# iden3/snarkjs

Measured on NVIDIA H100. Metric: groth16_proofs_per_sec, higher is better.
Workload: dtype u32x8 (256-bit modular integers, 32-bit limbs)

## Files before the change

snarkjs_b200/csrc/api.cu:

```cuda
#include <cstdio>
#include <cstdlib>
#include <cstring>
#include <string>
#include <vector>
#include <map>
#include <algorithm>
#include <mutex>
#include <future>
#include <thread>
#include <dlfcn.h>
#include <nccl.h>
#include <fcntl.h>
#include <unistd.h>
#include <sys/mman.h>
#include <sys/stat.h>
#include "../../include/snarkb200.h"
#include "ec.cuh"
#include "msm.cuh"
#include "msm_entry.h"
#include "fr_entry.h"

using namespace sb;
namespace sb { double calibrate(int what, cudaStream_t stream); extern int g_ntt_tile_log; }

// ... 272 lines not shown
        hex_to_mont<BnFq>("1", c->gen1.data()); hex_to_mont<BnFq>("2", c->gen1.data() + 32);
        hex_to_mont<BnFq>("1800deef121f1e76426a00665e5c4479674322d4f75edadd46debd5cd992f6ed", c->gen2.data());
        hex_to_mont<BnFq>("198e9393920d483a7260bfb731fb5d25f1aa493335a9e71297e485b7aef312c2", c->gen2.data() + 32);
        hex_to_mont<BnFq>("12c85ea5db8c6deb4aab71808dcb408fe3d1e7690c43d37b4ce6cc0166fa7daa", c->gen2.data() + 64);
        hex_to_mont<BnFq>("090689d0585ff075ec9e99ad690c3395bc4b313370b38ef355acdadcd122975b", c->gen2.data() + 96);
    } else {
        c->gen1.resize(96); c->gen2.resize(192);
        hex_to_mont<BlsFq>("17f1d3a73197d7942695638c4fa9ac0fc3688c4f9774b905a14e3a3f171bac586c55e83ff97a1aeffb3af00adb22c6bb", c->gen1.data());
        hex_to_mont<BlsFq>("08b3f481e3aaa0f1a09e30ed741d8ae4fcf5e095d5d00af600db18cb2c04b3edd03cc744a2888ae40caa232946c5e7e1", c->gen1.data() + 48);
        hex_to_mont<BlsFq>("024aa2b2f08f0a91260805272dc51051c6e47ad4fa403b02b4510b647ae3d1770bac0326a805bbefd48056c8c121bdb8", c->gen2.data());
        hex_to_mont<BlsFq>("13e02b6052719f607dacd3a088274f65596bd0d09920b61ab5da61bbdc7f5049334cf11213945d57e5ac7d055d042b7e", c->gen2.data() + 48);
        hex_to_mont<BlsFq>("0ce5d527727d6e118cc9cdc6da2e351aadfd9baa8cbdd3a76d429a695160d12c923ac9cc3baca289e193548608b82801", c->gen2.data() + 96);
        hex_to_mont<BlsFq>("0606c4a02ea734cc32acd2b02bc28b99cb3e287e85a763af267492ab572e99ab3f370d275cec1da1aaa9075ff05f79be", c->gen2.data() + 144);
    }
}

void prof_begin(sb_ctx* c) { c->stats.ev = c->prof_ev; c->stats.nev = 256; c->stats.used = 0; for (double& d : c->stat) d = 0; }
void prof_end(sb_ctx* c) {
    for (int i = 0; i + 1 < c->stats.used; i += 2) {
        float ms = 0; if (cudaEventElapsedTime(&ms, c->prof_ev[i], c->prof_ev[i + 1]) != cudaSuccess) { cudaGetLastError(); continue; }
        const int g = c->stats.tag[i / 2];
        if (g == PROF_ACC_G1) { c->stat[0] += ms; c->stat[2] += 1; c->stat[9] += ms; }
        else if (g == PROF_ACC_G2) { c->stat[1] += ms; c->stat[3] += 1; c->stat[10] += ms; }
        else if (g == PROF_SORT) c->stat[8] += ms;
        else if (g >= PROF_FOLD && g <= PROF_JOIN) c->stat[11 + (g - PROF_FOLD)] += ms;
    }
    c->stats.ev = nullptr; c->stats.used = 0;
}

int g_serial_prove = 0;
int g_no_tables = 0;
int g_msm_chunk_log = 0;

bool want_precomp(sb_ctx* c, uint64_t n) {
    if (g_no_tables || n < (1ull << 12)) return false;
    MsmGeom g = msm_geometry_precomp(n, 32, c->fr_bits);
    return (uint64_t)g.W * n < (1ull << 31);
}
int build_table(sb_ctx* c, const GroupOps& G, const void* d_bases, uint64_t n, void** table, MsmGeom* gp) {
    MsmGeom g = msm_geometry_precomp(n, 32, c->fr_bits);
    cudaError_t e = cudaMalloc(table, (size_t)g.W * n * G.aff_bytes);
    if (e != cudaSuccess) { *table = nullptr; return cuda_fail(c, e, "precompute table allocation"); }
    int rc = G.precompute(d_bases, n, g.c, g.W, *table, c->stream); c->launches++;
    if (rc) return cuda_fail(c, (cudaError_t)rc, "k_precompute");
    e = cudaStreamSynchronize(c->stream);
    if (e != cudaSuccess) return cuda_fail(c, e, "k_precompute");
    *gp = g;
    return 0;
}

void tick(sb_ctx* c, int i) { cudaEventRecord(c->ev[i], c->stream); }
float elapsed(sb_ctx* c, int a, int b) { float ms = 0; cudaEventElapsedTime(&ms, c->ev[a], c->ev[b]); return ms; }

int msm_dev_accumulate(sb_ctx* c, const GroupOps& G, const void* d_bases, const uint8_t* d_scalars, uint32_t sbytes, uint64_t n,
                       uint8_t* acc_xyzz, const MsmGeom* gp = nullptr, uint64_t first = 0) {
    const uint64_t MAXC = 1ull << (g_msm_chunk_log > 0 ? g_msm_chunk_log : 23);
    for (uint64_t off = 0; off < n; off += MAXC) {
        uint64_t cn = std::min(MAXC, n - off);
        MsmGeom g = msm_geometry(cn, sbytes, c->fr_bits);
        if (gp) {
            g = *gp; g.first = first + off; g.W = (int)((8 * sbytes + 1 + g.c - 1) / g.c);
        }
        MsmSorted s;
        int rc = msm_sort_entries(d_scalars + off * sbytes, sbytes, cn, g, c->sort_scratch, c->stream, &s, &c->stats);
        if (rc) return cuda_fail(c, (cudaError_t)rc, "msm_sort_entries");
        void* d_wsum = c->io[3].get((size_t)g.wsum_points() * G.xyzz_bytes);
// ... 75 lines not shown
    for (void* p : {k->tA, k->tB1, k->tB2, k->tC, k->tH, k->dA, k->dB1, k->dB2, k->dC, k->dH, (void*)k->d_rowptr, (void*)k->d_sig, k->d_coef, k->dW, k->dA_T, k->dB_T, k->dC_T, k->dTmp, k->dTmp2, k->dTmp3, k->dWsum})
        if (p) cudaFree(p);
    delete k;
}

template <class PR> static void fr_from_mont_bytes(const uint8_t* in, uint8_t* out) { Fp<PR> a; memcpy(&a, in, 32); a = Fp<PR>::from_mont(a); memcpy(out, &a, 32); }
template <class PR> static void fr_neg_mul_bytes(const uint8_t* r, const uint8_t* s, uint8_t* out) { Fp<PR> a, b; memcpy(&a, r, 32); memcpy(&b, s, 32); a = Fp<PR>::neg(Fp<PR>::mul(a, b)); memcpy(out, &a, 32); }

}

extern "C" {

const char* sb_version(void) { return "snarkb200 0.2 (sm_90a)"; }
int sb_comm_destroy(sb_ctx* c);

int sb_create(int curve, int device_id, sb_ctx** out) {
    if (!out || (curve != SB_BN254 && curve != SB_BLS12_381)) return SB_ERR_ARG;
    int ndev = 0;
    if (cudaGetDeviceCount(&ndev) != cudaSuccess || ndev == 0) return SB_ERR_NODEVICE;
    if (device_id < 0 || device_id >= ndev) return SB_ERR_ARG;
    if (cudaSetDevice(device_id) != cudaSuccess) return SB_ERR_CUDA;
    sb_ctx* c = new sb_ctx();
    c->curve = curve; c->device = device_id;
    c->n8q = curve == SB_BN254 ? 32 : 48;
    c->fr_bits = curve == SB_BN254 ? 254 : 255;
    if (curve == SB_BN254) { c->g1 = SB_GROUP_OPS(bn254_g1, 64); c->g2 = SB_GROUP_OPS(bn254_g2, 128); }
    else { c->g1 = SB_GROUP_OPS(bls12381_g1, 96); c->g2 = SB_GROUP_OPS(bls12381_g2, 192); }
    if (cudaStreamCreate(&c->stream) != cudaSuccess) { delete c; return SB_ERR_CUDA; }
    for (auto& e : c->ev) cudaEventCreate(&e);
    for (auto& e : c->prof_ev) cudaEventCreate(&e);
    for (auto& e : c->pev) cudaEventCreateWithFlags(&e, cudaEventDisableTiming);
    { int lo = 0, hi = 0; cudaDeviceGetStreamPriorityRange(&lo, &hi);
      for (auto& st : c->aux) cudaStreamCreateWithPriority(&st, cudaStreamDefault, hi); }
    if (cudaHostAlloc((void**)&c->pinned, 256 * 1024, cudaHostAllocDefault) != cudaSuccess) c->pinned = nullptr;
    for (int i = 0; i < 2; i++) { if (cudaHostAlloc((void**)&c->stage[i], STAGE_BYTES, cudaHostAllocDefault) != cudaSuccess) c->stage[i] = nullptr; cudaEventCreateWithFlags(&c->stage_ev[i], cudaEventDisableTiming); }
    init_generators(c);
    int rc = curve == SB_BN254 ? init_roots<BnFr>(c) : init_roots<BlsFr>(c);
    if (rc == 0 && fr_configure(curve) != 0) rc = SB_ERR_CUDA;
    if (rc) { sb_destroy(c); return rc; }
    *out = c;
    return SB_OK;
}

void sb_destroy(sb_ctx* c) {
    if (!c) return;
    sb_comm_destroy(c);
    cudaSetDevice(c->device);
    cudaStreamSynchronize(c->stream);
    for (auto* k : c->keys) if (k) free_key(k);
    for (auto* k : c->plonk_keys) if (k) plonk_free_key(k);
    for (auto* k : c->fflonk_keys) if (k) fflonk_free_key(k);
    for (auto& b : c->bases) { if (b.d) cudaFree(b.d); if (b.table) cudaFree(b.table); }
    for (auto* t : c->pre_cache) { t->lo.release(); t->hi.release(); delete t; }
    for (auto& kv : c->ntt_fwd) { kv.second.lo.release(); kv.second.hi.release(); }
    for (auto& kv : c->ntt_inv) { kv.second.lo.release(); kv.second.hi.release(); }
    for (auto& kv : c->ninv) kv.second.release();
    c->wr_fwd.release(); c->wr_inv.release();
    for (auto& b : c->io) b.release();
    c->sort_scratch.release(); c->bucket_scratch.release();
    for (auto& e : c->ev) cudaEventDestroy(e);
    for (auto& e : c->prof_ev) cudaEventDestroy(e);
    for (auto& e : c->pev) cudaEventDestroy(e);
    for (auto& st : c->aux) { if (st) { cudaStreamSynchronize(st); cudaStreamDestroy(st); } }
    if (c->pinned) cudaFreeHost(c->pinned);
    for (int i = 0; i < 2; i++) { if (c->stage[i]) cudaFreeHost(c->stage[i]); cudaEventDestroy(c->stage_ev[i]); }
    c->sort_scratch2.release(); for (auto& b : c->bscr) b.release();
    cudaStreamDestroy(c->stream);
// ... 320 lines not shown
    k->nCoef = ncoef;
    cudaError_t e = cudaSuccess;
    auto up = [&](void** d, const void* src, size_t bytes, size_t alloc) {
        if (e != cudaSuccess) return;
        e = cudaMalloc(d, alloc ? alloc : 16); if (e != cudaSuccess) return;
        if (bytes) e = cudaMemcpy(*d, src, bytes, cudaMemcpyHostToDevice);
    };
    k->shard = shard; k->n_shards = n_shards;
    sb_shard_range(nv, shard, n_shards, &k->wlo, &k->wcnt);
    sb_shard_range(n, shard, n_shards, &k->hlo, &k->hcnt);
    const uint64_t wlo = k->wlo, wcnt = k->wcnt, hlo = k->hlo, hcnt = k->hcnt;
    auto upsec = [&](void** d, uint32_t id, uint64_t off, uint64_t len) {
        if (e != cudaSuccess) return;
        e = cudaMalloc(d, len ? len : 16); if (e != cudaSuccess) return;
        e = zkey_to_device(c, src, secs, id, off, len, *d);
    };
    upsec(&k->dA, 5, wlo * sG1, wcnt * sG1);
    upsec(&k->dB1, 6, wlo * sG1, wcnt * sG1);
    upsec(&k->dB2, 7, wlo * sG2, wcnt * sG2);
    if (e == cudaSuccess) {
        const uint64_t np1 = (uint64_t)k->nPublic + 1;
        e = cudaMalloc(&k->dC, wcnt ? wcnt * sG1 : 16);
        if (e == cudaSuccess && wcnt) e = cudaMemset(k->dC, 0, wcnt * sG1);
        const uint64_t g0 = std::max(wlo, np1), g1 = wlo + wcnt;
        if (e == cudaSuccess && g1 > g0) e = zkey_to_device(c, src, secs, 8, (g0 - np1) * sG1, (g1 - g0) * sG1, (uint8_t*)k->dC + (g0 - wlo) * sG1);
    }
    upsec(&k->dH, 9, hlo * sG1, hcnt * sG1);
    up((void**)&k->d_rowptr, rowptr.data(), rowptr.size() * 8, rowptr.size() * 8);
    up((void**)&k->d_sig, sig.data(), (size_t)ncoef * 4, (size_t)ncoef * 4);
    up(&k->d_coef, coef.data(), (size_t)ncoef * 32, (size_t)ncoef * 32);
    up(&k->dW, nullptr, 0, (nv + 64) * 32);
    up(&k->dA_T, nullptr, 0, n * 32); up(&k->dB_T, nullptr, 0, n * 32); up(&k->dC_T, nullptr, 0, n * 32); up(&k->dTmp, nullptr, 0, n * 32);
    up(&k->dTmp2, nullptr, 0, n * 32); up(&k->dTmp3, nullptr, 0, n * 32);
    up(&k->dWsum, nullptr, 0, 8 * 80 * 4 * 96);
    if (e != cudaSuccess) { free_key(k); return cuda_fail(c, e, "sb_groth16_load upload"); }
    if (want_precomp(c, wcnt) && want_precomp(c, hcnt)) {
        int rc2 = build_table(c, c->g1, k->dA, wcnt, &k->tA, &k->gpW);
        if (!rc2) rc2 = build_table(c, c->g1, k->dB1, wcnt, &k->tB1, &k->gpW);
        if (!rc2) rc2 = build_table(c, c->g2, k->dB2, wcnt, &k->tB2, &k->gpW);
        if (!rc2) rc2 = build_table(c, c->g1, k->dC, wcnt, &k->tC, &k->gpW);
        if (!rc2) rc2 = build_table(c, c->g1, k->dH, hcnt, &k->tH, &k->gpH);
        if (rc2) { free_key(k); return rc2; }
    }
    c->keys.push_back(k);
    *handle = c->keys.size();
    return 0;
}

int sb_groth16_load(sb_ctx* c, const uint8_t* z, uint64_t zlen, uint64_t* handle) { SB_LOCK(c);
    if (!z) return SB_ERR_ARG;
    ZkeySource src; src.z = z; src.zlen = zlen; return groth16_load_impl(c, src, 0, 1, handle);
}
int sb_groth16_load_sharded(sb_ctx* c, const uint8_t* z, uint64_t zlen, int shard, int n_shards, uint64_t* handle) { SB_LOCK(c);
    if (!z) return SB_ERR_ARG;
    ZkeySource src; src.z = z; src.zlen = zlen; return groth16_load_impl(c, src, shard, n_shards, handle);
}

int sb_groth16_load_file(sb_ctx* c, const char* path, uint64_t* handle) { SB_LOCK(c);
    if (!c || !path) return SB_ERR_ARG;
    cudaSetDevice(c->device);
    FILE* f = fopen(path, "rb");
    if (!f) return fail(c, SB_ERR_FORMAT, std::string("cannot open ") + path);
    ZkeySource src; src.f = f;
    int rc = groth16_load_impl(c, src, 0, 1, handle);
    fclose(f);
    return rc;
}
// ... 172 lines not shown
                        if (qcnt) NC(c, nc, nc->Send((const uint8_t*)odd[j] + qlo * 32, qcnt * 32, ncclUint8, q, c->comm, c->stream));
                    }
                } else if (hcnt) NC(c, nc, nc->Recv((uint8_t*)odd[j] + hlo * 32, hcnt * 32, ncclUint8, o, c->comm, c->stream));
            }
            NC(c, nc, nc->GroupEnd());
        }
        if (hcnt) {
            ProfScope pj(&c->stats, PROF_JOIN, c->stream);
            rc = fr_join_abc(cv, (const uint8_t*)odd[0] + hlo * 32, (const uint8_t*)odd[1] + hlo * 32, (const uint8_t*)odd[2] + hlo * 32,
                             (uint8_t*)tmp + hlo * 32, hcnt, c->stream); c->launches++;
            pj.end();
            if (rc) return cuda_fail(c, (cudaError_t)rc, "fr_join_abc");
        }
        return 0;
    };
    const GroupOps& G1 = c->g1; const GroupOps& G2 = c->g2;
    uint8_t* pA = partials; uint8_t* pB1 = pA + G1.xyzz_bytes; uint8_t* pC = pB1 + G1.xyzz_bytes; uint8_t* pH = pC + G1.xyzz_bytes; uint8_t* pB2 = pH + G1.xyzz_bytes;
    memset(partials, 0, 4 * G1.xyzz_bytes + G2.xyzz_bytes);
    std::vector<uint8_t> sA(G1.xyzz_bytes, 0), rB1(G1.xyzz_bytes, 0);
    const uint64_t MAXC = 1ull << (g_msm_chunk_log > 0 ? g_msm_chunk_log : 23);
    const bool local = k->n_shards > 1;
    if (local && (shard != k->shard || n_shards != k->n_shards)) return fail(c, SB_ERR_ARG, "proving key was loaded for a different shard");
    const uint64_t wb = local ? 0 : wlo, hb = local ? 0 : hlo;
    const bool overlapped = wcnt <= MAXC && hcnt <= MAXC && wcnt > 0 && hcnt > 0 && c->pinned;
    if (dist && world > 1 && !overlapped) return fail(c, SB_ERR_ARG, "distributed proving needs at least one point per rank and shards of at most 2^23 points");
    if (overlapped) {
        const bool serial = g_serial_prove != 0;
        cudaStream_t s0 = c->stream;
        cudaStream_t sN = serial ? s0 : c->aux[5];
        MsmGeom gw = msm_geometry(wcnt, 32, c->fr_bits), gh = msm_geometry(hcnt, 32, c->fr_bits);
        const bool pre = k->tA != nullptr;
        if (pre) { gw = k->gpW; gw.first = wb; gh = k->gpH; gh.first = hb; }
        const size_t w1 = (size_t)gw.wsum_points() * G1.xyzz_bytes, w2 = (size_t)gw.wsum_points() * G2.xyzz_bytes, wh = (size_t)gh.wsum_points() * G1.xyzz_bytes;
        if (3 * w1 + w2 + wh + 64 > 256 * 1024 || 3 * w1 + w2 + wh > (size_t)8 * 80 * 4 * 96) return fail(c, SB_ERR_ARG, "window buffer too small");
        uint8_t* dws = (uint8_t*)k->dWsum; uint8_t* hws = c->pinned;
        uint64_t* hcounts = (uint64_t*)(c->pinned + 3 * w1 + w2 + wh);
        CU(c, cudaEventRecord(c->pev[0], s0));
        if (sN != s0) CU(c, cudaStreamWaitEvent(sN, c->pev[0], 0));
        cudaStream_t saved = c->stream; c->stream = sN;
        rc = run_qap_ntt();
        MsmSorted sh;
        if (!rc) { rc = msm_sort_entries((const uint8_t*)tmp + hlo * 32, 32, hcnt, gh, c->sort_scratch2, sN, &sh, &c->stats); if (rc) rc = cuda_fail(c, (cudaError_t)rc, "msm_sort_entries"); }
        c->stream = saved;
        if (rc) return rc;
        CU(c, cudaEventRecord(c->pev[1], sN));
        MsmSorted sw;
        rc = msm_sort_entries((const uint8_t*)k->dW + wlo * 32, 32, wcnt, gw, c->sort_scratch, s0, &sw, &c->stats);
        if (rc) return cuda_fail(c, (cudaError_t)rc, "msm_sort_entries");
        tick(c, 2);
        struct Job { const GroupOps* G; const void* bases; size_t off; size_t len; uint8_t* dst; int tag; const MsmSorted* srt; const MsmGeom* g; };
        Job jobs[5] = {{&G1, pre ? k->tA : (const void*)((const uint8_t*)k->dA + wb * G1.aff_bytes), 0, w1, pA, SB_G1, &sw, &gw},
                       {&G1, pre ? k->tB1 : (const void*)((const uint8_t*)k->dB1 + wb * G1.aff_bytes), w1, w1, pB1, SB_G1, &sw, &gw},
                       {&G2, pre ? k->tB2 : (const void*)((const uint8_t*)k->dB2 + wb * G2.aff_bytes), 3 * w1, w2, pB2, SB_G2, &sw, &gw},
                       {&G1, pre ? k->tC : (const void*)((const uint8_t*)k->dC + wb * G1.aff_bytes), 2 * w1, w1, pC, SB_G1, &sw, &gw},
                       {&G1, pre ? k->tH : (const void*)((const uint8_t*)k->dH + hb * G1.aff_bytes), 3 * w1 + w2, wh, pH, SB_G1, &sh, &gh}};
        for (int i = 0; i < 5; i++) {
            cudaStream_t st = serial ? s0 : c->aux[i];
            if (i == 4 && sN != s0) CU(c, cudaStreamWaitEvent(s0, c->pev[1], 0));
            c->stats.cur_tag = jobs[i].tag;
            rc = jobs[i].G->buckets(jobs[i].bases, *jobs[i].srt, c->bscr[i], s0, dws + jobs[i].off, &c->stats, st, c->pev[8 + i]);
            if (rc) return cuda_fail(c, (cudaError_t)rc, "msm_buckets");
            CU(c, cudaMemcpyAsync(hws + jobs[i].off, dws + jobs[i].off, jobs[i].len, cudaMemcpyDeviceToHost, st));
            if (i == 0) CU(c, cudaMemcpyAsync(&hcounts[0], sw.counts, 8, cudaMemcpyDeviceToHost, st));
            if (i == 4) CU(c, cudaMemcpyAsync(&hcounts[1], sh.counts, 8, cudaMemcpyDeviceToHost, st));
            CU(c, cudaEventRecord(c->pev[2 + i], st));
        }
        tick(c, 3);
        for (int i = 0; i < 5; i++) {
            CU(c, cudaEventSynchronize(c->pev[2 + i]));
            jobs[i].G->combine(hws + jobs[i].off, *jobs[i].g, jobs[i].dst);
            if (ps && i == 0) G1.times(pA, ps->sp, 32, sA.data());
            if (ps && i == 1) G1.times(pB1, ps->rp, 32, rB1.data());
        }
        if (!serial) { for (int i = 0; i < 5; i++) CU(c, cudaStreamWaitEvent(s0, c->pev[2 + i], 0)); CU(c, cudaStreamWaitEvent(s0, c->pev[1], 0)); }
        c->stat[4] += 3.0 * (double)hcounts[0] + (double)hcounts[1]; c->stat[5] += (double)hcounts[0];
    } else {
    rc = run_qap_ntt(); if (rc) return rc;
    tick(c, 2);
    for (uint64_t off = 0; off < wcnt; off += MAXC) {
        uint64_t cn = std::min(MAXC, wcnt - off), base = wb + off;
        MsmGeom g = msm_geometry(cn, 32, c->fr_bits);
        MsmSorted s;
        rc = msm_sort_entries((const uint8_t*)k->dW + (wlo + off) * 32, 32, cn, g, c->sort_scratch, c->stream, &s, &c->stats);
        if (rc) return cuda_fail(c, (cudaError_t)rc, "msm_sort_entries");
        uint8_t* ws = (uint8_t*)k->dWsum;
        size_t w1 = (size_t)g.wsum_points() * G1.xyzz_bytes, w2 = (size_t)g.wsum_points() * G2.xyzz_bytes;
        if (3 * w1 + w2 > (size_t)8 * 80 * 4 * 96) return fail(c, SB_ERR_ARG, "window buffer too small");
        c->stats.cur_tag = SB_G1;
        rc = G1.buckets((const uint8_t*)k->dA + base * G1.aff_bytes, s, c->bucket_scratch, c->stream, ws, &c->stats, nullptr, nullptr); if (rc) return cuda_fail(c, (cudaError_t)rc, "msm A");
        rc = G1.buckets((const uint8_t*)k->dB1 + base * G1.aff_bytes, s, c->bucket_scratch, c->stream, ws + w1, &c->stats, nullptr, nullptr); if (rc) return cuda_fail(c, (cudaError_t)rc, "msm B1");
        rc = G1.buckets((const uint8_t*)k->dC + base * G1.aff_bytes, s, c->bucket_scratch, c->stream, ws + 2 * w1, &c->stats, nullptr, nullptr); if (rc) return cuda_fail(c, (cudaError_t)rc, "msm C");
        c->stats.cur_tag = SB_G2;
        rc = G2.buckets((const uint8_t*)k->dB2 + base * G2.aff_bytes, s, c->bucket_scratch, c->stream, ws + 3 * w1, &c->stats, nullptr, nullptr); if (rc) return cuda_fail(c, (cudaError_t)rc, "msm B2");
        std::vector<uint8_t> hw(3 * w1 + w2);
        uint64_t entries = 0;
        CU(c, cudaMemcpyAsync(hw.data(), ws, hw.size(), cudaMemcpyDeviceToHost, c->stream));
        CU(c, cudaMemcpyAsync(&entries, s.counts, 8, cudaMemcpyDeviceToHost, c->stream));
        CU(c, cudaStreamSynchronize(c->stream));
        c->stat[4] += 3.0 * (double)entries; c->stat[5] += (double)entries;
        G1.combine(hw.data(), g, pA); G1.combine(hw.data() + w1, g, pB1); G1.combine(hw.data() + 2 * w1, g, pC); G2.combine(hw.data() + 3 * w1, g, pB2);
    }
    tick(c, 3);
    if (hcnt) {
        rc = msm_dev_accumulate(c, G1, (const uint8_t*)k->dH + hb * G1.aff_bytes, (const uint8_t*)tmp + hlo * 32, 32, hcnt, pH);
        if (rc) return rc;
    }
    if (ps) { G1.times(pA, ps->sp, 32, sA.data()); G1.times(pB1, ps->rp, 32, rB1.data()); }
    }
    if (ps) {
        G1.add(pC, pH); G1.add(pC, sA.data()); G1.add(pC, rB1.data());
        memset(pB1, 0, G1.xyzz_bytes); memset(pH, 0, G1.xyzz_bytes);
    }
    tick(c, 4);
    cudaEventSynchronize(c->ev[4]);
    prof_end(c);
    c->last_ms[0] = elapsed(c, 0, 4); c->last_ms[1] = elapsed(c, 0, 1); c->last_ms[2] = elapsed(c, 1, 2); c->last_ms[3] = elapsed(c, 2, 3); c->last_ms[4] = elapsed(c, 3, 4);
    return 0;
}


// ... 332 lines not shown
```

snarkjs_b200/csrc/msm.cuh:

```cuda
#pragma once
#include <cuda_runtime.h>
#include "ec.cuh"
#include "msm_geom.h"

namespace sb {

static constexpr int MSM_SEG = 32;
static constexpr int MSM_ACC_THREADS = 128;
static constexpr int MSM_RED_CHUNK = 16;
static constexpr uint32_t MSM_INVALID_KEY = 0xffffffffu;
static constexpr int MSM_COUNTS_SEG = 8;

extern int g_msm_force_c;

__host__ inline MsmGeom msm_choose(uint64_t n, uint32_t scalar_bytes, int fr_bits, bool precomp) {
    int eff = (int)(8 * scalar_bytes) < fr_bits ? (int)(8 * scalar_bytes) : fr_bits;
    int best_c = 3; double best = 1e300;
    for (int c = 3; c <= 22; c++) {
        int weff = (eff + 1 + c - 1) / c, top = eff + 1 - (weff - 1) * c;
        if (weff > 1 && top < c - 5) continue;
        double buckets = (precomp ? 1.0 : (double)weff) * (double)(1u << (c - 1));
        double cost = (double)weff * (double)n * 10.0 + buckets * 60.0;
        if (cost < best) { best = cost; best_c = c; }
    }
// ... 185 lines not shown
    for (uint32_t s = 16; s > 0; s >>= 1) {
        if (threadIdx.x < s) { XYZZ<F> a = load_vec(sm + threadIdx.x), b = load_vec(sm + threadIdx.x + s); a.add(b); store_vec(sm + threadIdx.x, a); }
        __syncwarp();
    }
    if (threadIdx.x == 0) store_vec(out + blockIdx.x, load_vec(sm));
}

template <class F> __device__ __noinline__ void padd(XYZZ<F>& a, const XYZZ<F>& b) { a.add(b); }

struct AxisJob { const void* in; void* out; uint64_t total; uint32_t S; uint32_t log_inner; };

template <class F>
__global__ void __launch_bounds__(128)
k_axis_sum(AxisJob j0, AxisJob j1) {
    const AxisJob j = blockIdx.y ? j1 : j0;
    const uint64_t gid = blockIdx.x * (uint64_t)blockDim.x + threadIdx.x;
    if (gid >= j.total) return;
    const uint64_t o = gid >> j.log_inner, i = gid & ((1ull << j.log_inner) - 1);
    const XYZZ<F>* p = (const XYZZ<F>*)j.in + ((o * j.S) << j.log_inner) + i;
    XYZZ<F> acc = load_vec(p);
#pragma unroll 1
    for (uint32_t s = 1; s < j.S; s++) { XYZZ<F> v = load_vec(p + ((uint64_t)s << j.log_inner)); acc.add(v); }
    store_vec((XYZZ<F>*)j.out + gid, acc);
}

template <class F> __device__ __forceinline__ XYZZ<F> shfl_down_pt(const XYZZ<F>& v, int d) {
    constexpr int NW32 = sizeof(XYZZ<F>) / 4;
    union U { XYZZ<F> p; uint32_t w[NW32]; __device__ U() {} };
    U a, r; a.p = v;
#pragma unroll
    for (int k = 0; k < NW32; k++) r.w[k] = __shfl_down_sync(0xffffffffu, a.w[k], d);
    return r.p;
}
template <class F> __device__ __forceinline__ void warp_weighted_sum(XYZZ<F> v, XYZZ<F>& T, XYZZ<F>& W) {
    const int lane = threadIdx.x & 31;
#pragma unroll 1
    for (int d = 1; d < 32; d <<= 1) { XYZZ<F> o = shfl_down_pt<F>(v, d); if (lane + d < 32) v.add(o); }
    T = v;
    XYZZ<F> x = lane ? v : XYZZ<F>::inf();
#pragma unroll 1
    for (int d = 16; d >= 1; d >>= 1) { XYZZ<F> o = shfl_down_pt<F>(x, d); if (lane < d) x.add(o); }
    W = x;
}
template <class F> __device__ __forceinline__ XYZZ<F> warp_sum(XYZZ<F> x) {
    const int lane = threadIdx.x & 31;
#pragma unroll 1
    for (int d = 16; d >= 1; d >>= 1) { XYZZ<F> o = shfl_down_pt<F>(x, d); if (lane < d) x.add(o); }
    return x;
}

template <class F>
__global__ void __launch_bounds__(128)
k_ws_chunks(const XYZZ<F>* __restrict__ vecR, uint32_t lenR, const XYZZ<F>* __restrict__ vecC, uint32_t lenC, uint32_t NW, XYZZ<F>* __restrict__ tw) {
    const uint32_t nR = (lenR + 31) / 32, nC = (lenC + 31) / 32, per = nR + nC;
    const uint32_t wid = blockIdx.x * (blockDim.x >> 5) + (threadIdx.x >> 5), lane = threadIdx.x & 31;
    if (wid >= NW * per) return;
    const uint32_t w = wid / per, jj = wid % per;
    const bool isR = jj < nR;
    const uint32_t j = isR ? jj : jj - nR, len = isR ? lenR : lenC, idx = j * 32 + lane;
    const XYZZ<F>* vec = (isR ? vecR : vecC) + (uint64_t)w * len;
    XYZZ<F> v = XYZZ<F>::inf();
    if (idx < len) v = load_vec(vec + idx);
    XYZZ<F> T, W;
    warp_weighted_sum<F>(v, T, W);
    if (lane == 0) { store_vec(tw + 2 * (uint64_t)wid, T); store_vec(tw + 2 * (uint64_t)wid + 1, W); }
}

template <class F>
__global__ void __launch_bounds__(128)
k_ws_final(const XYZZ<F>* __restrict__ tw, uint32_t nR, uint32_t nC, XYZZ<F>* __restrict__ out) {
    const uint32_t warp = threadIdx.x >> 5, lane = threadIdx.x & 31, per = nR + nC;
    const XYZZ<F>* base = tw + 2 * (uint64_t)blockIdx.x * per;
    const bool r_side = warp < 2;
    const uint32_t cnt = r_side ? nR : nC, off = r_side ? 0 : nR;
    XYZZ<F> v = XYZZ<F>::inf();
    if (lane < cnt) v = load_vec(base + 2 * (uint64_t)(off + lane) + (warp & 1));
    XYZZ<F>* o = out + 5 * (uint64_t)blockIdx.x;
    if ((warp & 1) == 0) {
        XYZZ<F> tot, res;
        warp_weighted_sum<F>(v, tot, res);
        if (lane == 0) { store_vec(o + (r_side ? 0 : 2), res); if (!r_side) store_vec(o + 4, tot); }
    } else {
        XYZZ<F> res = warp_sum<F>(v);
        if (lane == 0) store_vec(o + (r_side ? 1 : 3), res);
    }
}

template <class F>
__global__ void __launch_bounds__(128)
k_axis_tree(AxisJob j0, AxisJob j1) {
    const AxisJob j = blockIdx.y ? j1 : j0;
    const uint64_t wid = blockIdx.x * (uint64_t)(blockDim.x >> 5) + (threadIdx.x >> 5);
    const uint32_t lane = threadIdx.x & 31;
    if (wid >= j.total) return;
    const uint64_t o = wid >> j.log_inner, i = wid & ((1ull << j.log_inner) - 1);
    const XYZZ<F>* p = (const XYZZ<F>*)j.in + ((o * j.S) << j.log_inner) + i;
    XYZZ<F> acc = XYZZ<F>::inf();
#pragma unroll 1
    for (uint32_t s = lane; s < j.S; s += 32) { XYZZ<F> v = load_vec(p + ((uint64_t)s << j.log_inner)); acc.add(v); }
    acc = warp_sum<F>(acc);
    if (lane == 0) store_vec((XYZZ<F>*)j.out + wid, acc);
}

static constexpr int WS_COL_BITS = 10;
struct WsPlan {
    bool ok = false;
    int m = 0, er = 0, ec = 0;
    int levels = 0; int br[8] = {0}, bc[8] = {0};
    uint32_t lenR = 0, lenC = 0, nR = 0, nC = 0;
    size_t rowA = 0, rowB = 0, colA = 0, colB = 0, tw = 0;
    size_t elems() const { return rowA + rowB + colA + colB + tw + 8; }
};
__host__ inline WsPlan ws_plan(const MsmGeom& g) {
    WsPlan p; const int cbits = g.c - 1; const size_t NW = g.windows();
    if (cbits > 2 * WS_COL_BITS || cbits < 0) return p;
    p.ok = true;
    if (cbits > WS_COL_BITS) { p.m = WS_COL_BITS; p.er = p.m; p.ec = cbits - p.m; p.lenR = 1u << p.ec; p.lenC = 1u << p.m; }
    else { p.lenR = 0; p.lenC = g.B; }
    int rr = p.er, rc = p.ec;
    for (int l = 0; l < 2 && (rr > 0 || rc > 0); l++) {
        p.levels++;
        p.br[l] = l == 0 ? (rr < 3 ? rr : 3) : rr; p.bc[l] = l == 0 ? (rc < 3 ? rc : 3) : rc; rr -= p.br[l]; rc -= p.bc[l];
        const size_t orow = p.br[l] ? (NW * g.B) >> (p.er - rr) : 0, ocol = p.bc[l] ? (NW * g.B) >> (p.ec - rc) : 0;
        if (l & 1) { p.rowB = orow; p.colB = ocol; } else { p.rowA = orow; p.colA = ocol; }
    }
    p.nR = (p.lenR + 31) / 32; p.nC = (p.lenC + 31) / 32;
    p.tw = 2 * NW * (p.nR + p.nC);
    return p;
}
__host__ inline size_t msm_reduce_scratch_elems(const MsmGeom& g) {
    const uint32_t NW = g.windows();
    const uint32_t L = g.B < (uint32_t)MSM_RED_CHUNK ? g.B : MSM_RED_CHUNK;
    const uint32_t ctas_per_window = (g.B / L + 127) / 128;
    const size_t legacy = (size_t)2 * NW * ctas_per_window;
    const WsPlan p = ws_plan(g);
    return (p.ok && p.elems() > legacy) ? p.elems() : legacy;
}

template <class F>
__global__ void __launch_bounds__(128) k_precompute(const Affine<F>* __restrict__ bases, uint64_t n, int c, int W, Affine<F>* __restrict__ table) {
    uint64_t i = blockIdx.x * (uint64_t)blockDim.x + threadIdx.x;
    if (i >= n) return;
    Affine<F> a = load_vec(bases + i);
    store_vec(table + i, a);
    if (a.is_inf()) {
        for (int w = 1; w < W; w++) store_vec(table + (uint64_t)w * n + i, a);
        return;
    }
    XYZZ<F> p; p.x = a.x; p.y = a.y; p.zz = F::one(); p.zzz = F::one();
    for (int w = 1; w < W; w++) {
        for (int j = 0; j < c; j++) p = XYZZ<F>::dbl(p);
        Affine<F> o;
        if (p.is_inf()) { o.x = F::zero(); o.y = F::zero(); }
        else { F t = PairInvF(F::mul(p.zz, p.zzz)); o.x = F::mul(p.x, F::mul(t, p.zzz)); o.y = F::mul(p.y, F::mul(t, p.zz)); p.x = o.x; p.y = o.y; p.zz = F::one(); p.zzz = F::one(); }
        store_vec(table + (uint64_t)w * n + i, o);
    }
}

__host__ __device__ inline uint64_t splitmix64(uint64_t x) {
    x += 0x9E3779B97F4A7C15ull; x = (x ^ (x >> 30)) * 0xBF58476D1CE4E5B9ull; x = (x ^ (x >> 27)) * 0x94D049BB133111EBull; return x ^ (x >> 31);
// ... 86 lines not shown
        ProfScope prof(stats, stats ? stats->cur_tag : 0, stream);
        {
            const unsigned grid = (unsigned)((heads0 + MSM_ACC_THREADS - 1) / MSM_ACC_THREADS);
            constexpr int MINB = sizeof(F) > 32 ? 2 : 4;
            k_accumulate<F, MINB><<<grid, MSM_ACC_THREADS, 0, stream>>>(d_bases, s.keys, s.vals, s.counts, buckets, headsA, hkA);
            launches++;
        }
        prof.end();
        if (tail_stream && tail_stream != stream && ev_acc) {
            cudaEventRecord(ev_acc, stream); cudaStreamWaitEvent(tail_stream, ev_acc, 0); stream = tail_stream;
        }
        ProfScope pfold(stats, PROF_FOLD, stream);
        k_fold_short<F><<<(unsigned)((heads0 + MSM_ACC_THREADS - 1) / MSM_ACC_THREADS), MSM_ACC_THREADS, 0, stream>>>(
            headsA, hkA, hkM, s.counts, buckets); launches++;
        uint64_t m = heads0; int level = 1;
        XYZZ<F>* hin = headsA; uint32_t* kin = hkM; XYZZ<F>* hout = headsB; uint32_t* kout = hkB;
        while (true) {
            uint64_t threads = (m + MSM_SEG - 1) / MSM_SEG;
            k_fold<F><<<(unsigned)((threads + MSM_ACC_THREADS - 1) / MSM_ACC_THREADS), MSM_ACC_THREADS, 0, stream>>>(
                hin, kin, s.counts, level, buckets, hout, kout); launches++;
            if (m <= (uint64_t)MSM_SEG) break;
            m = threads; level++;
            XYZZ<F>* th = hin; hin = hout; hout = th; uint32_t* tk = kin; kin = kout; kout = tk;
            if (level >= 8) return (int)cudaErrorUnknown;
        }
        pfold.end();
    }
    if (!heads0 && tail_stream && tail_stream != stream && ev_acc) { cudaEventRecord(ev_acc, stream); cudaStreamWaitEvent(tail_stream, ev_acc, 0); stream = tail_stream; }
    ProfScope pred(stats, PROF_REDUCE, stream);
    const WsPlan wp = ws_plan(g);
    if (wp.ok && !g_msm_force_reduce) {
        XYZZ<F>* rowb[2] = {partials, partials + wp.rowA};
        XYZZ<F>* colb[2] = {partials + wp.rowA + wp.rowB, partials + wp.rowA + wp.rowB + wp.colA};
        XYZZ<F>* tw = partials + wp.rowA + wp.rowB + wp.colA + wp.colB;
        const XYZZ<F>* rin = buckets; const XYZZ<F>* cin = buckets;
        int rr = wp.er, rc = wp.ec;
        for (int l = 0; l < wp.levels; l++) {
            AxisJob jr{nullptr, nullptr, 0, 1, 0}, jc{nullptr, nullptr, 0, 1, 0};
            if (wp.br[l]) { rr -= wp.br[l]; jr = AxisJob{rin, rowb[l & 1], (uint64_t)nbuckets >> (wp.er - rr), 1u << wp.br[l], (uint32_t)rr}; rin = rowb[l & 1]; }
            if (wp.bc[l]) { rc -= wp.bc[l]; jc = AxisJob{cin, colb[l & 1], (uint64_t)nbuckets >> (wp.ec - rc), 1u << wp.bc[l], (uint32_t)wp.m}; cin = colb[l & 1]; }
            const uint64_t mx = jr.total > jc.total ? jr.total : jc.total;
            if (l == 0) k_axis_sum<F><<<dim3((unsigned)((mx + 127) / 128), 2), 128, 0, stream>>>(jr, jc);
            else k_axis_tree<F><<<dim3((unsigned)((mx + 3) / 4), 2), 128, 0, stream>>>(jr, jc);
            launches++;
        }
        const uint32_t per = wp.nR + wp.nC;
        k_ws_chunks<F><<<(NW * per + 3) / 4, 128, 0, stream>>>(wp.lenR ? rin : nullptr, wp.lenR, cin, wp.lenC, NW, tw); launches++;
        k_ws_final<F><<<NW, 128, 0, stream>>>(tw, wp.nR, wp.nC, d_wsum); launches++;
    } else {
        k_reduce<F><<<NW * ctas_per_window, red_threads, red_threads * sizeof(XYZZ<F>), stream>>>(buckets, g, partials, ctas_per_window); launches++;
        k_window_sum<F><<<NW, 32, 32 * sizeof(XYZZ<F>), stream>>>(partials, ctas_per_window, d_wsum); launches++;
    }
    pred.end();
    if (stats) stats->launches += launches;
    return (int)cudaGetLastError();
}

}
```

snarkjs_b200/csrc/msm_geom.h:

```cpp
#pragma once
#include <cstdint>
namespace sb {
struct MsmGeom {
    int c;
    int W;
    uint32_t B;
    int precomp = 0;
    uint64_t stride = 0, first = 0;
    uint32_t windows() const { return precomp ? 1u : (uint32_t)W; }
    uint32_t wsum_points() const { return 5u * windows(); }
};
}
```

snarkjs_b200/csrc/msm_sort.cu:

```cuda
#include <cub/device/device_radix_sort.cuh>
#include "msm.cuh"

namespace sb {

int g_msm_force_reduce = 0;
int g_msm_force_c = 0;

__global__ void k_digits(const uint8_t* __restrict__ scalars, uint32_t sbytes, uint64_t n, MsmGeom g,
                         uint32_t* __restrict__ keys, uint32_t* __restrict__ vals) {
    uint64_t i = blockIdx.x * (uint64_t)blockDim.x + threadIdx.x;
    if (i >= n) return;
    uint32_t w32[17];
    const uint8_t* s = scalars + i * sbytes;
    if (sbytes == 32 && ((uintptr_t)scalars & 15) == 0) {
        const uint4* p = reinterpret_cast<const uint4*>(s);
        uint4 a = __ldg(p), b = __ldg(p + 1);
        w32[0] = a.x; w32[1] = a.y; w32[2] = a.z; w32[3] = a.w; w32[4] = b.x; w32[5] = b.y; w32[6] = b.z; w32[7] = b.w;
#pragma unroll
        for (int k = 8; k < 17; k++) w32[k] = 0;
    } else {
#pragma unroll
        for (int k = 0; k < 17; k++) w32[k] = 0;
        for (uint32_t k = 0; k < sbytes; k++) w32[k >> 2] |= (uint32_t)s[k] << (8 * (k & 3));
    }
    const uint32_t cmask = (1u << g.c) - 1, half = 1u << (g.c - 1);
    uint32_t carry = 0;
    for (int w = 0; w < g.W; w++) {
        uint32_t bit = (uint32_t)w * g.c, wi = bit >> 5, sh = bit & 31;
        uint64_t two = (uint64_t)w32[wi] | ((uint64_t)(wi + 1 < 17 ? w32[wi + 1] : 0) << 32);
        uint32_t raw = ((uint32_t)(two >> sh) & cmask) + carry;
        uint32_t key, val = (uint32_t)i;
        if (raw > half) { raw = (1u << g.c) - raw; carry = 1; val |= 0x80000000u; } else carry = 0;
        if (g.precomp) { key = raw ? raw - 1 : MSM_INVALID_KEY; val = (uint32_t)((uint64_t)w * g.stride + g.first + i) | (val & 0x80000000u); }
        else key = raw ? (uint32_t)w * g.B + raw - 1 : MSM_INVALID_KEY;
        keys[(uint64_t)w * n + i] = key;
        vals[(uint64_t)w * n + i] = val;
    }
}

__global__ void k_count_valid(const uint32_t* __restrict__ keys, uint64_t total, uint64_t* __restrict__ out, uint32_t T, uint32_t seg_lo, uint64_t wave) {
    if (blockIdx.x | threadIdx.x) return;
    uint64_t lo = 0, hi = total;
    while (lo < hi) { uint64_t mid = (lo + hi) >> 1; if (keys[mid] == MSM_INVALID_KEY) hi = mid; else lo = mid + 1; }
    out[0] = lo;
    uint64_t seg = T;
    if (wave) {
        const uint64_t k = (lo + wave * T - 1) / (wave * T);
        if (k && k <= 3) seg = (lo + k * wave - 1) / (k * wave);
        if (seg < seg_lo) seg = seg_lo;
        if (seg > T) seg = T;
    }
    out[MSM_COUNTS_SEG] = seg;
    uint64_t m = (lo + seg - 1) / seg;
    out[1] = m;
    for (int l = 2; l < 8; l++) { m = (m <= MSM_SEG) ? 0 : (m + MSM_SEG - 1) / MSM_SEG; out[l] = m; }
}

int msm_sort_entries(const uint8_t* d_scalars, uint32_t sbytes, uint64_t n, MsmGeom g, MsmScratch& scratch,
                     cudaStream_t stream, MsmSorted* out, MsmLaunchStats* stats) {
    const uint64_t total = n * (uint64_t)g.W;
    const uint64_t nbuckets = (uint64_t)g.windows() * g.B;
    if (sbytes == 0 || sbytes > 64) return (int)cudaErrorInvalidValue;
    int key_bits = 1; while ((1ull << key_bits) < nbuckets) key_bits++;
    int end_bit = key_bits + 1 > 32 ? 32 : key_bits + 1;
    size_t sort_tmp = 0;
    cub::DoubleBuffer<uint32_t> kb(nullptr, nullptr), vb(nullptr, nullptr);
    cub::DeviceRadixSort::SortPairs(nullptr, sort_tmp, kb, vb, (uint64_t)total, 0, end_bit, stream);
    auto al = [](size_t x) { return (x + 255) & ~(size_t)255; };
    size_t o_keys0 = 0, o_keys1 = o_keys0 + al(total * 4), o_vals0 = o_keys1 + al(total * 4), o_vals1 = o_vals0 + al(total * 4);
    size_t o_tmp = o_vals1 + al(total * 4), o_counts = o_tmp + al(sort_tmp);
    uint8_t* base = (uint8_t*)scratch.get(o_counts + 256);
    if (!base) return (int)cudaErrorMemoryAllocation;
    uint32_t* keys0 = (uint32_t*)(base + o_keys0); uint32_t* keys1 = (uint32_t*)(base + o_keys1);
    uint32_t* vals0 = (uint32_t*)(base + o_vals0); uint32_t* vals1 = (uint32_t*)(base + o_vals1);
    uint64_t* counts = (uint64_t*)(base + o_counts);
    int launches = 0;
    ProfScope prof(stats, PROF_SORT, stream);
    k_digits<<<(unsigned)((n + 255) / 256), 256, 0, stream>>>(d_scalars, sbytes, n, g, keys0, vals0); launches++;
    kb = cub::DoubleBuffer<uint32_t>(keys0, keys1); vb = cub::DoubleBuffer<uint32_t>(vals0, vals1);
    cudaError_t e = cub::DeviceRadixSort::SortPairs(base + o_tmp, sort_tmp, kb, vb, (uint64_t)total, 0, end_bit, stream);
    if (e != cudaSuccess) return (int)e;
    launches += 2 + (end_bit + 7) / 8;
    uint32_t T = MSM_SEG;
// ... 16 lines not shown
```

Measured before the change: 34.09.

## Replace weighted window sum with per-bit bucket sums and cap segment waves

Replaces the two-kernel weighted running-sum bucket reduction (k_ws_chunks + k_ws_final) with a single k_bit_sums kernel. For each window it computes the total plus one partial sum per bucket-index bit, giving c points per window instead of 5. The host-side window-sum buffers grow to 512 KiB to hold the larger output, so the host must combine more points. Separately, when the sorted entry count exceeds three waves, the segment length is now sized to fill exactly three waves instead of staying at T, which changes accumulation load balance. A profiling script is also added.

```diff
diff --git a/profiles/prof_tail.py b/profiles/prof_tail.py
--- /dev/null
+++ b/profiles/prof_tail.py
@@ -0,0 +1,68 @@
+import collections
+import os
+import re
+import sys
+
+sys.path.insert(0, os.path.dirname(os.path.dirname(os.path.abspath(__file__))))
+import numpy as np
+import torch
+from torch.profiler import ProfilerActivity, profile
+
+import snarkjs_b200
+from snarkjs_b200 import groth16, synth
+from snarkjs_b200.curve import _ptr
+
+FOLD = ("k_fold_short", "k_fold")
+REDUCE = ("k_axis_sum", "k_axis_tree", "k_bit_sums", "k_ws_chunks", "k_ws_final", "k_reduce", "k_window_sum")
+
+
+def short_name(name: str) -> str:
+    m = re.search(r"(\w+)\s*(<|\()", re.sub(r"^void\s+", "", name))
+    base = m.group(1) if m else name[:60]
+    return base + (" [G2]" if "Fp2" in name else "")
+
+
+def main():
+    L = int(os.environ.get("LOGN", "20"))
+    c = snarkjs_b200.getCurveFromName("bn128")
+    c.lib.sb_set_tuning(2, 1)
+    pk = groth16.ProvingKey(synth.synth_groth16_zkey(c, L, seed=1), curve=c)
+    w = synth.chain_witness(c.r, L)
+    r = (5 * (1 << 256) % c.r).to_bytes(32, "little")
+    s = (7 * (1 << 256) % c.r).to_bytes(32, "little")
+    proof = np.empty(8 * c.n8q, np.uint8)
+
+    def prove():
+        c.check(c.lib.sb_groth16_prove(c.handle, pk.handle, _ptr(w), w.size // 32, r, s, _ptr(proof)))
+
+    for _ in range(3):
+        prove()
+    torch.cuda.synchronize()
+    with profile(activities=[ProfilerActivity.CUDA]) as prof:
+        prove()
+        torch.cuda.synchronize()
+    tot = collections.defaultdict(float)
+    cnt = collections.defaultdict(int)
+    for e in prof.events():
+        if e.device_type != torch.autograd.DeviceType.CUDA:
+            continue
+        k = short_name(e.name)
+        tot[k] += e.time_range.elapsed_us() / 1e3
+        cnt[k] += 1
+    if not tot:
+        raise SystemExit("torch.profiler recorded no CUDA kernels")
+    gpu = torch.cuda.get_device_name(0)
+    print(f"# {gpu}, Groth16 2^{L}, serialised, prove call {c.last_ms(0):.2f} ms (library events)")
+    print(f"{'kernel':<44}{'ms':>9}{'launches':>10}")
+    for k in sorted(tot, key=tot.get, reverse=True):
+        print(f"{k:<44}{tot[k]:9.3f}{cnt[k]:10d}")
+    print(f"{'total kernel time':<44}{sum(tot.values()):9.3f}{sum(cnt.values()):10d}")
+    for label, names in (("fold", FOLD), ("bucket_reduce", REDUCE)):
+        ms = sum(v for k, v in tot.items() if k.split(" ")[0] in names)
+        n = sum(v for k, v in cnt.items() if k.split(" ")[0] in names)
+        print(f"class {label:<38}{ms:9.3f}{n:10d}")
+    pk.release()
+
+
+if __name__ == "__main__":
+    main()
diff --git a/snarkjs_b200/csrc/api.cu b/snarkjs_b200/csrc/api.cu
--- a/snarkjs_b200/csrc/api.cu
+++ b/snarkjs_b200/csrc/api.cu
@@ -328,6 +328,8 @@
 int g_no_tables = 0;
 int g_msm_chunk_log = 0;
 
+static constexpr size_t WSUM_BYTES = 512 * 1024;
+
 bool want_precomp(sb_ctx* c, uint64_t n) {
     if (g_no_tables || n < (1ull << 12)) return false;
     MsmGeom g = msm_geometry_precomp(n, 32, c->fr_bits);
@@ -469,7 +471,7 @@
     for (auto& e : c->pev) cudaEventCreateWithFlags(&e, cudaEventDisableTiming);
     { int lo = 0, hi = 0; cudaDeviceGetStreamPriorityRange(&lo, &hi);
       for (auto& st : c->aux) cudaStreamCreateWithPriority(&st, cudaStreamDefault, hi); }
-    if (cudaHostAlloc((void**)&c->pinned, 256 * 1024, cudaHostAllocDefault) != cudaSuccess) c->pinned = nullptr;
+    if (cudaHostAlloc((void**)&c->pinned, WSUM_BYTES, cudaHostAllocDefault) != cudaSuccess) c->pinned = nullptr;
     for (int i = 0; i < 2; i++) { if (cudaHostAlloc((void**)&c->stage[i], STAGE_BYTES, cudaHostAllocDefault) != cudaSuccess) c->stage[i] = nullptr; cudaEventCreateWithFlags(&c->stage_ev[i], cudaEventDisableTiming); }
     init_generators(c);
     int rc = curve == SB_BN254 ? init_roots<BnFr>(c) : init_roots<BlsFr>(c);
@@ -856,7 +858,7 @@
     up(&k->dW, nullptr, 0, (nv + 64) * 32);
     up(&k->dA_T, nullptr, 0, n * 32); up(&k->dB_T, nullptr, 0, n * 32); up(&k->dC_T, nullptr, 0, n * 32); up(&k->dTmp, nullptr, 0, n * 32);
     up(&k->dTmp2, nullptr, 0, n * 32); up(&k->dTmp3, nullptr, 0, n * 32);
-    up(&k->dWsum, nullptr, 0, 8 * 80 * 4 * 96);
+    up(&k->dWsum, nullptr, 0, WSUM_BYTES);
     if (e != cudaSuccess) { free_key(k); return cuda_fail(c, e, "sb_groth16_load upload"); }
     if (want_precomp(c, wcnt) && want_precomp(c, hcnt)) {
         int rc2 = build_table(c, c->g1, k->dA, wcnt, &k->tA, &k->gpW);
@@ -1095,7 +1097,7 @@
         const bool pre = k->tA != nullptr;
         if (pre) { gw = k->gpW; gw.first = wb; gh = k->gpH; gh.first = hb; }
         const size_t w1 = (size_t)gw.wsum_points() * G1.xyzz_bytes, w2 = (size_t)gw.wsum_points() * G2.xyzz_bytes, wh = (size_t)gh.wsum_points() * G1.xyzz_bytes;
-        if (3 * w1 + w2 + wh + 64 > 256 * 1024 || 3 * w1 + w2 + wh > (size_t)8 * 80 * 4 * 96) return fail(c, SB_ERR_ARG, "window buffer too small");
+        if (3 * w1 + w2 + wh + 64 > WSUM_BYTES) return fail(c, SB_ERR_ARG, "window buffer too small");
         uint8_t* dws = (uint8_t*)k->dWsum; uint8_t* hws = c->pinned;
         uint64_t* hcounts = (uint64_t*)(c->pinned + 3 * w1 + w2 + wh);
         CU(c, cudaEventRecord(c->pev[0], s0));
@@ -1148,7 +1150,7 @@
         if (rc) return cuda_fail(c, (cudaError_t)rc, "msm_sort_entries");
         uint8_t* ws = (uint8_t*)k->dWsum;
         size_t w1 = (size_t)g.wsum_points() * G1.xyzz_bytes, w2 = (size_t)g.wsum_points() * G2.xyzz_bytes;
-        if (3 * w1 + w2 > (size_t)8 * 80 * 4 * 96) return fail(c, SB_ERR_ARG, "window buffer too small");
+        if (3 * w1 + w2 > WSUM_BYTES) return fail(c, SB_ERR_ARG, "window buffer too small");
         c->stats.cur_tag = SB_G1;
         rc = G1.buckets((const uint8_t*)k->dA + base * G1.aff_bytes, s, c->bucket_scratch, c->stream, ws, &c->stats, nullptr, nullptr); if (rc) return cuda_fail(c, (cudaError_t)rc, "msm A");
         rc = G1.buckets((const uint8_t*)k->dB1 + base * G1.aff_bytes, s, c->bucket_scratch, c->stream, ws + w1, &c->stats, nullptr, nullptr); if (rc) return cuda_fail(c, (cudaError_t)rc, "msm B1");
diff --git a/snarkjs_b200/csrc/msm.cuh b/snarkjs_b200/csrc/msm.cuh
--- a/snarkjs_b200/csrc/msm.cuh
+++ b/snarkjs_b200/csrc/msm.cuh
@@ -241,16 +241,6 @@
     for (int k = 0; k < NW32; k++) r.w[k] = __shfl_down_sync(0xffffffffu, a.w[k], d);
     return r.p;
 }
-template <class F> __device__ __forceinline__ void warp_weighted_sum(XYZZ<F> v, XYZZ<F>& T, XYZZ<F>& W) {
-    const int lane = threadIdx.x & 31;
-#pragma unroll 1
-    for (int d = 1; d < 32; d <<= 1) { XYZZ<F> o = shfl_down_pt<F>(v, d); if (lane + d < 32) v.add(o); }
-    T = v;
-    XYZZ<F> x = lane ? v : XYZZ<F>::inf();
-#pragma unroll 1
-    for (int d = 16; d >= 1; d >>= 1) { XYZZ<F> o = shfl_down_pt<F>(x, d); if (lane < d) x.add(o); }
-    W = x;
-}
 template <class F> __device__ __forceinline__ XYZZ<F> warp_sum(XYZZ<F> x) {
     const int lane = threadIdx.x & 31;
 #pragma unroll 1
@@ -260,39 +250,32 @@
 
 template <class F>
 __global__ void __launch_bounds__(128)
-k_ws_chunks(const XYZZ<F>* __restrict__ vecR, uint32_t lenR, const XYZZ<F>* __restrict__ vecC, uint32_t lenC, uint32_t NW, XYZZ<F>* __restrict__ tw) {
-    const uint32_t nR = (lenR + 31) / 32, nC = (lenC + 31) / 32, per = nR + nC;
-    const uint32_t wid = blockIdx.x * (blockDim.x >> 5) + (threadIdx.x >> 5), lane = threadIdx.x & 31;
-    if (wid >= NW * per) return;
-    const uint32_t w = wid / per, jj = wid % per;
-    const bool isR = jj < nR;
-    const uint32_t j = isR ? jj : jj - nR, len = isR ? lenR : lenC, idx = j * 32 + lane;
-    const XYZZ<F>* vec = (isR ? vecR : vecC) + (uint64_t)w * len;
-    XYZZ<F> v = XYZZ<F>::inf();
-    if (idx < len) v = load_vec(vec + idx);
-    XYZZ<F> T, W;
-    warp_weighted_sum<F>(v, T, W);
-    if (lane == 0) { store_vec(tw + 2 * (uint64_t)wid, T); store_vec(tw + 2 * (uint64_t)wid + 1, W); }
-}
-
-template <class F>
-__global__ void __launch_bounds__(128)
-k_ws_final(const XYZZ<F>* __restrict__ tw, uint32_t nR, uint32_t nC, XYZZ<F>* __restrict__ out) {
-    const uint32_t warp = threadIdx.x >> 5, lane = threadIdx.x & 31, per = nR + nC;
-    const XYZZ<F>* base = tw + 2 * (uint64_t)blockIdx.x * per;
-    const bool r_side = warp < 2;
-    const uint32_t cnt = r_side ? nR : nC, off = r_side ? 0 : nR;
-    XYZZ<F> v = XYZZ<F>::inf();
-    if (lane < cnt) v = load_vec(base + 2 * (uint64_t)(off + lane) + (warp & 1));
-    XYZZ<F>* o = out + 5 * (uint64_t)blockIdx.x;
-    if ((warp & 1) == 0) {
-        XYZZ<F> tot, res;
-        warp_weighted_sum<F>(v, tot, res);
-        if (lane == 0) { store_vec(o + (r_side ? 0 : 2), res); if (!r_side) store_vec(o + 4, tot); }
-    } else {
-        XYZZ<F> res = warp_sum<F>(v);
-        if (lane == 0) store_vec(o + (r_side ? 1 : 3), res);
-    }
+k_bit_sums(const XYZZ<F>* __restrict__ vecR, int ec, const XYZZ<F>* __restrict__ vecC, int m, XYZZ<F>* __restrict__ out) {
+    extern __shared__ uint4 smem_raw[];
+    XYZZ<F>* sm = reinterpret_cast<XYZZ<F>*>(smem_raw);
+    const uint32_t per = 1 + m + ec, w = blockIdx.x / per, j = blockIdx.x % per;
+    const bool isR = j > (uint32_t)m;
+    const int bits = isR ? ec : m, k = isR ? (int)j - 1 - m : (int)j - 1;
+    const XYZZ<F>* vec = isR ? vecR + ((uint64_t)w << ec) : vecC + ((uint64_t)w << m);
+    const uint32_t terms = j == 0 ? 1u << m : 1u << (bits - 1);
+    XYZZ<F> acc = XYZZ<F>::inf();
+#pragma unroll 1
+    for (uint32_t i = threadIdx.x; i < terms; i += blockDim.x) {
+        const uint32_t idx = j == 0 ? i : ((i >> k) << (k + 1)) | (1u << k) | (i & ((1u << k) - 1));
+        XYZZ<F> v = load_vec(vec + idx);
+        acc.add(v);
+    }
+    store_vec(sm + threadIdx.x, acc);
+    __syncthreads();
+    for (uint32_t s = blockDim.x >> 1; s > 0; s >>= 1) {
+        if (threadIdx.x < s) {
+            XYZZ<F> a = load_vec(sm + threadIdx.x), b = load_vec(sm + threadIdx.x + s);
+            a.add(b);
+            store_vec(sm + threadIdx.x, a);
+        }
+        __syncthreads();
+    }
+    if (threadIdx.x == 0) store_vec(out + blockIdx.x, load_vec(sm));
 }
 
 template <class F>
@@ -316,16 +299,15 @@
     bool ok = false;
     int m = 0, er = 0, ec = 0;
     int levels = 0; int br[8] = {0}, bc[8] = {0};
-    uint32_t lenR = 0, lenC = 0, nR = 0, nC = 0;
-    size_t rowA = 0, rowB = 0, colA = 0, colB = 0, tw = 0;
-    size_t elems() const { return rowA + rowB + colA + colB + tw + 8; }
+    size_t rowA = 0, rowB = 0, colA = 0, colB = 0;
+    size_t elems() const { return rowA + rowB + colA + colB + 8; }
 };
 __host__ inline WsPlan ws_plan(const MsmGeom& g) {
     WsPlan p; const int cbits = g.c - 1; const size_t NW = g.windows();
     if (cbits > 2 * WS_COL_BITS || cbits < 0) return p;
     p.ok = true;
-    if (cbits > WS_COL_BITS) { p.m = WS_COL_BITS; p.er = p.m; p.ec = cbits - p.m; p.lenR = 1u << p.ec; p.lenC = 1u << p.m; }
-    else { p.lenR = 0; p.lenC = g.B; }
+    if (cbits > WS_COL_BITS) { p.m = WS_COL_BITS; p.er = p.m; p.ec = cbits - p.m; }
+    else p.m = cbits;
     int rr = p.er, rc = p.ec;
     for (int l = 0; l < 2 && (rr > 0 || rc > 0); l++) {
         p.levels++;
@@ -333,8 +315,6 @@
         const size_t orow = p.br[l] ? (NW * g.B) >> (p.er - rr) : 0, ocol = p.bc[l] ? (NW * g.B) >> (p.ec - rc) : 0;
         if (l & 1) { p.rowB = orow; p.colB = ocol; } else { p.rowA = orow; p.colA = ocol; }
     }
-    p.nR = (p.lenR + 31) / 32; p.nC = (p.lenC + 31) / 32;
-    p.tw = 2 * NW * (p.nR + p.nC);
     return p;
 }
 __host__ inline size_t msm_reduce_scratch_elems(const MsmGeom& g) {
@@ -487,7 +467,6 @@
     if (wp.ok && !g_msm_force_reduce) {
         XYZZ<F>* rowb[2] = {partials, partials + wp.rowA};
         XYZZ<F>* colb[2] = {partials + wp.rowA + wp.rowB, partials + wp.rowA + wp.rowB + wp.colA};
-        XYZZ<F>* tw = partials + wp.rowA + wp.rowB + wp.colA + wp.colB;
         const XYZZ<F>* rin = buckets; const XYZZ<F>* cin = buckets;
         int rr = wp.er, rc = wp.ec;
         for (int l = 0; l < wp.levels; l++) {
@@ -499,9 +478,7 @@
             else k_axis_tree<F><<<dim3((unsigned)((mx + 3) / 4), 2), 128, 0, stream>>>(jr, jc);
             launches++;
         }
-        const uint32_t per = wp.nR + wp.nC;
-        k_ws_chunks<F><<<(NW * per + 3) / 4, 128, 0, stream>>>(wp.lenR ? rin : nullptr, wp.lenR, cin, wp.lenC, NW, tw); launches++;
-        k_ws_final<F><<<NW, 128, 0, stream>>>(tw, wp.nR, wp.nC, d_wsum); launches++;
+        k_bit_sums<F><<<NW * (1 + wp.m + wp.ec), 128, 128 * sizeof(XYZZ<F>), stream>>>(rin, wp.ec, cin, wp.m, d_wsum); launches++;
     } else {
         k_reduce<F><<<NW * ctas_per_window, red_threads, red_threads * sizeof(XYZZ<F>), stream>>>(buckets, g, partials, ctas_per_window); launches++;
         k_window_sum<F><<<NW, 32, 32 * sizeof(XYZZ<F>), stream>>>(partials, ctas_per_window, d_wsum); launches++;
diff --git a/snarkjs_b200/csrc/msm_geom.h b/snarkjs_b200/csrc/msm_geom.h
--- a/snarkjs_b200/csrc/msm_geom.h
+++ b/snarkjs_b200/csrc/msm_geom.h
@@ -8,6 +8,6 @@
     int precomp = 0;
     uint64_t stride = 0, first = 0;
     uint32_t windows() const { return precomp ? 1u : (uint32_t)W; }
-    uint32_t wsum_points() const { return 5u * windows(); }
+    uint32_t wsum_points() const { return (uint32_t)c * windows(); }
 };
 }
diff --git a/snarkjs_b200/csrc/msm_sort.cu b/snarkjs_b200/csrc/msm_sort.cu
--- a/snarkjs_b200/csrc/msm_sort.cu
+++ b/snarkjs_b200/csrc/msm_sort.cu
@@ -38,6 +38,8 @@
     }
 }
 
+static constexpr uint64_t MSM_BIG_WAVES = 3;
+
 __global__ void k_count_valid(const uint32_t* __restrict__ keys, uint64_t total, uint64_t* __restrict__ out, uint32_t T, uint32_t seg_lo, uint64_t wave) {
     if (blockIdx.x | threadIdx.x) return;
     uint64_t lo = 0, hi = total;
@@ -46,9 +48,13 @@
     uint64_t seg = T;
     if (wave) {
         const uint64_t k = (lo + wave * T - 1) / (wave * T);
-        if (k && k <= 3) seg = (lo + k * wave - 1) / (k * wave);
-        if (seg < seg_lo) seg = seg_lo;
-        if (seg > T) seg = T;
+        if (k && k <= 3) {
+            seg = (lo + k * wave - 1) / (k * wave);
+            if (seg < seg_lo) seg = seg_lo;
+            if (seg > T) seg = T;
+        } else if (k > 3) {
+            seg = (lo + MSM_BIG_WAVES * wave - 1) / (MSM_BIG_WAVES * wave);
+        }
     }
     out[MSM_COUNTS_SEG] = seg;
     uint64_t m = (lo + seg - 1) / seg;
```

After: 34.58, median of 6. +1.5%, better.
